# AnyLoc/Revisit-Anything

Measured on AMD Instinct MI355X. Metric: query_images_per_sec, higher is better.
Workload: dtype f32

## Files before the change

revisit-anything_amd/csrc/ctx.h:

```cpp
#pragma once
#include <hip/hip_runtime.h>
#include <math.h>
#include <stdint.h>
#include <stdio.h>
#include <string.h>

#include <map>
#include <string>
#include <vector>

#include "../../include/segvlad.h"

#define SV_HIP(expr)                                                                              \
  do {                                                                                            \
    hipError_t _e = (expr);                                                                       \
    if (_e != hipSuccess) {                                                                       \
      return ctx->fail(SEGVLAD_ERR_HIP, "%s failed: %s (%s:%d)", #expr, hipGetErrorString(_e),    \
                       __FILE__, __LINE__);                                                       \
    }                                                                                             \
  } while (0)

#define SV_TRY(expr)          \
  do {                        \
    int _r = (expr);          \
// ... 277 lines not shown
  if (ctx->desc.open)                                                                                                       \
  return ctx->fail(SEGVLAD_ERR_STATE, what ": a segvlad_describe_begin is open on this context (call segvlad_describe_end first)")

StageTimer* sv_stage_open(segvlad_ctx* ctx, const char* name, int* slot);
struct StageScope {
  segvlad_ctx* ctx;
  StageTimer* t = nullptr;
  int slot = 0;
  StageScope(segvlad_ctx* c, const char* name) : ctx(c) { t = sv_stage_open(c, name, &slot); }
  ~StageScope() { if (t) (void)hipEventRecord(t->ev[2 * slot + 1], ctx->stream); }
  void count(int n = 1) { if (t) t->launches += n; }
};

int sv_launch_vocab_prepare(segvlad_ctx* ctx);
int sv_launch_incidence(segvlad_ctx* ctx, const uint8_t* masks, int S, int Hm, int Wm, int H, int W, int patch,
                        uint64_t* inc_bits, double* centroids );
int sv_launch_centroids(segvlad_ctx* ctx, const uint8_t* masks, int S, int Hm, int Wm, double* out);
bool sv_adjacency_fits(int S_max);
int sv_launch_adjacency(segvlad_ctx* ctx, const double* cent, const int32_t* seg_off_dev, const int64_t* adj_off_dev,
                        int B, int S_max, int order, uint8_t* adj, uint32_t* n_bad, uint8_t* img_flags = nullptr);
int sv_launch_assign(segvlad_ctx* ctx, const float* tokens, int B, int N, float* xt, uint8_t* labels, float* rnorm,
                     float* gap);
int sv_launch_prep(segvlad_ctx* ctx, const uint8_t* labels, const uint64_t* inc_bits, const int32_t* seg_off_dev,
                   const int64_t* adj_off_dev, const uint8_t* adj, int B, int N, int K, int S_max, int SC,
                   uint64_t* colmask, float* gscale, int32_t* phys , int32_t* cov_cnt ,
                   int cover );
int sv_launch_aggregate(segvlad_ctx* ctx, const float* xt, const float* rnorm, const uint8_t* labels,
                        const uint64_t* colmask, const float* centres, int K, int D, const int32_t* seg_off_dev,
                        const float* gscale, int B, int N, int SC, float* out, float* block_norms,
                        const float* mean = nullptr, float xscale = 0.f, uint16_t* h1 = nullptr, uint16_t* h2 = nullptr);

int sv_launch_token_norms(segvlad_ctx* ctx, const float* xt, const uint64_t* colmask, const float* centres, int K, int D,
                          const int32_t* seg_off_dev, int B, int N, int SC, float* block_norms, float xscale, uint16_t* h1,
                          uint16_t* h2, const int32_t* rowbase, int64_t dummy_row ,
                          const int32_t* phys );

int sv_launch_centroid_sums(segvlad_ctx* ctx, const float* xt, const float* rnorm, const uint8_t* labels, int B, int N, int D, int K,
                            double* sums, int64_t* counts);

int sv_launch_row_sumsq(segvlad_ctx* ctx, const float* X, int64_t n, int d, float* out);
int sv_launch_normalize_rows(segvlad_ctx* ctx, const float* X, int64_t n, int d, float* Y);
int sv_launch_gemm_nt(segvlad_ctx* ctx, int mode, const float* A, const float* Bm, float* C, int M, int N, int Kd,
                      int64_t ldc, const float* a_sub, const float* col_scale, const float* row_add,
                      const float* col_add);

int sv_launch_l2_strided(segvlad_ctx* ctx, const float* Q, const float* R, float* dist, int M, int n_sample, int Kd,
                         int64_t ldc, const float* qn, const float* rn, int b_stride, bool split_ok = false);
int sv_launch_l2_strided_parts(segvlad_ctx* ctx, const float* Q, const float* R, float* dist, int M, int n_sample, int Kd,
                               int64_t ldc, const float* qn, const float* rn, int b_stride, const float** parts, int* splits);
int sv_launch_l0_reduce_rank(segvlad_ctx* ctx, const float* parts, int splits, int M, int n_sample, int64_t ldc, const float* qn,
                             const float* rn, int b_stride, int rank, float* thr_out, uint32_t* cand_cnt, const uint32_t* fail_rows);
int sv_launch_l2_filter(segvlad_ctx* ctx, const float* Q, const float* R, int M, int n_sample, int Kd, const float* qn,
                        const float* rn, int b_stride, const float* thr, int64_t thr_ld, uint32_t* cand_cnt,
                        float* cand_d2, uint32_t* cand_id, int cap);

int sv_launch_split_bf16(segvlad_ctx* ctx, const float* X, int64_t n_elems, uint16_t* hi, uint16_t* lo);
int sv_launch_bf16_filter(segvlad_ctx* ctx, const uint16_t* Qh, const uint16_t* Ql, const uint16_t* Rh, const uint16_t* Rl,
                          int M, int n_sample, int d, int b_stride, const float* qn, const float* rn, const float* thr,
                          int64_t thr_ld, float eps_mult, float c_eps, float rn_max, uint32_t* cand_cnt, float* cand_d2,
                          uint32_t* cand_id, int cap);
enum class SvSelect : int { Threshold = 0, Band = 1, Carry = 2 };
struct SvSelectArgs {
  uint32_t* cnt = nullptr;
  float* cd2 = nullptr;
  uint32_t* cid = nullptr;
  int cap = 0;
  int k = 0;
  SvSelect mode = SvSelect::Threshold;
// ... 132 lines not shown
```

revisit-anything_amd/csrc/describe.hip:

```cpp
#include <cmath>
#include "ctx.h"


struct SegWalk { int S_max = 0; bool monotone = true; std::vector<int64_t> adj_off; };
static SegWalk walk_seg_offsets(const int32_t* seg_offsets, int B) {
  SegWalk w;
  w.adj_off.assign((size_t)B + 1, 0);
  for (int b = 0; b < B && w.monotone; ++b) {
    const int s = seg_offsets[b + 1] - seg_offsets[b];
    w.monotone = s >= 0;
    if (s > w.S_max) w.S_max = s;
    w.adj_off[b + 1] = w.adj_off[b] + (int64_t)s * s;
  }
  return w;
}

static int incidence_run(segvlad_ctx* ctx, const uint8_t* masks, int S, int Hm, int Wm, int H, int W, int patch, uint64_t* inc_bits,
                         double* centroids, bool want_centroids) {
  if (S < 0 || Hm <= 0 || Wm <= 0 || H <= 0 || W <= 0 || patch <= 0 || H / patch <= 0 || W / patch <= 0)
    return ctx->fail(SEGVLAD_ERR_ARG, "incidence: bad geometry S=%d masks %dx%d image %dx%d patch %d", S, Hm, Wm, H, W, patch);
  if (S == 0) return SEGVLAD_OK;
  if (!masks || !inc_bits || (want_centroids && !centroids)) return ctx->fail(SEGVLAD_ERR_ARG, "incidence: null pointer");
  const int N = (H / patch) * (W / patch), nw = (N + 63) / 64;
  const void* dm;
// ... 93 lines not shown
  SegWalk w = walk_seg_offsets(io.seg_offsets, B);
  if (!w.monotone) return PLAN_REFUSE(SEGVLAD_ERR_ARG, "images: seg_offsets must be non-decreasing");
  p.S_tot = io.seg_offsets[B], p.S_max = w.S_max, p.SC = w.S_max > 0 ? (w.S_max + 63) / 64 : 1;
  p.adj_off = std::move(w.adj_off);
  const bool plain = pca && !x3;
  const float* y = plain ? nullptr : io.y;
  if (p.S_tot > 0 && (!io.inc_bits || (!io.out && !y && !plain))) return PLAN_REFUSE(SEGVLAD_ERR_ARG, "images: null inc_bits/out");
  p.upload_offsets = passes == Passes::All;
  p.want_desc = p.S_tot > 0 && (io.out || plain), p.want_block_norms = io.block_norms_out && p.S_tot > 0;
  p.want_labels = io.labels_out != nullptr, p.want_gap = io.gap_out != nullptr;
  p.want_y = y != nullptr && p.S_tot > 0;
  if (plain) p.form = DescribeForm::PlainProjection;
  if (!p.want_y) return p;
  const bool project = io.out == nullptr && D % 32 == 0 && ctx->P % 4 == 0 && ctx->opt.pca_path != 1 &&
                       (ctx->opt.pca_path == 2 || ((double)p.S_tot * K >= 1.25 * (double)B * N && (double)B * N >= 128.0 * K));
  p.form = project ? DescribeForm::Project : DescribeForm::Planes;
  p.xscale = sv_fp16_scale(1.f + ctx->pca_mean_maxabs);
  if (!project) return p;
  const float bound = 1.f + ctx->vocab_maxabs;
  if (!std::isfinite(bound)) return PLAN_REFUSE(SEGVLAD_ERR_ARG, "images_pca: the vocabulary holds a non-finite centre");
  p.xscale = sv_fp16_scale(bound);
  p.rows_pad = (((int64_t)B * N + 255) & ~255ll) + 256ll * K;
  if (ctx->pca_w_scale > 0.f) {
    const float zb = std::sqrt((float)D) * (16384.f / ctx->pca_w_scale) * (1.f + ctx->vocab_norm_max);
    if (std::isfinite(zb) && zb > 0.f) p.zscale = sv_fp16_scale(zb);
  }
  return p;
#undef PLAN_REFUSE
}

static int reserve_scratch(segvlad_ctx* ctx, const DescribePlan& p, DescribeIO& io) {
  const size_t B = p.B, N = p.N, D = p.D, K = p.K, P = p.P, S = p.S_tot;
  if (p.form == DescribeForm::Project) {
    SV_HIP(ctx->s_xh1.reserve((size_t)(p.rows_pad + 256) * D * 2));
    SV_HIP(ctx->s_xh2.reserve((size_t)(p.rows_pad + 256) * D * 2));
    SV_HIP(ctx->s_pz.reserve((size_t)p.rows_pad * P * sizeof(float)));
    SV_HIP(ctx->s_rowbase.reserve(B * K * sizeof(int32_t)));
    SV_HIP(ctx->s_tilegrp.reserve((size_t)(p.rows_pad >> 8) * sizeof(int32_t)));
    SV_HIP(ctx->s_phys.reserve(B * N * sizeof(int32_t)));
    SV_HIP(ctx->s_covcnt.reserve(B * K * sizeof(int32_t)));
    SV_HIP(ctx->s_bn.reserve(S * K * sizeof(float)));
  } else if (p.form == DescribeForm::Planes) {
    SV_HIP(ctx->s_xh1.reserve((size_t)sv_x3_rows(p.S_tot) * ctx->KD * 2));
    SV_HIP(ctx->s_xh2.reserve((size_t)sv_x3_rows(p.S_tot) * ctx->KD * 2));
  } else if (p.form == DescribeForm::PlainProjection && !io.out && S > 0) {
    SV_HIP(ctx->s_desc.reserve(S * ctx->KD * sizeof(float)));
    io.out = ctx->s_desc.as<float>();
  }
  SV_HIP(ctx->s_xt.reserve(B * N * D * sizeof(float)));
  SV_HIP(ctx->s_rnorm.reserve(B * N * sizeof(float)));
  if (!p.want_labels) SV_HIP(ctx->s_labels.reserve(B * N));
  if (p.passes == Passes::AssignOnly) return SEGVLAD_OK;
  SV_HIP(ctx->s_colmask.reserve(B * N * p.SC * 8));
  SV_HIP(ctx->s_gscale.reserve((S + 1) * sizeof(float)));
  SV_HIP(ctx->s_segoff.reserve((B + 1) * sizeof(int32_t)));
  SV_HIP(ctx->s_adjoff.reserve((B + 1) * sizeof(int64_t)));
  return SEGVLAD_OK;
}

static int stage_pointers(segvlad_ctx* ctx, const DescribePlan& p, DescribeIO& io) {
  const size_t B = p.B, N = p.N, S = p.S_tot;
  if (p.want_y) SV_TRY(sv_out(ctx, io.y, S * p.P * sizeof(float), &io.d_y));
  SV_TRY(sv_in(ctx, io.tokens, B * p.D * N * sizeof(float), &io.d_tok));
  if (S > 0) SV_TRY(sv_in(ctx, io.inc_bits, S * p.nw * 8, &io.d_inc));
  if (io.adj && S > 0) SV_TRY(sv_in(ctx, io.adj, (size_t)p.adj_off[B], &io.d_adj));
  if (p.want_desc) SV_TRY(sv_out(ctx, io.out, S * p.K * p.D * sizeof(float), &io.d_out));
  if (p.want_labels) SV_TRY(sv_out(ctx, io.labels_out, B * N, &io.d_lab));
  else io.d_lab = ctx->s_labels.p;
// ... 27 lines not shown
  if (!p.l2norm) return SEGVLAD_OK;
  SV_TRY(sv_launch_normalize_rows(ctx, (const float*)io.d_y, p.S_tot, p.P, (float*)io.d_y));
  sc.count();
  return SEGVLAD_OK;
}

static int pass_descriptor(segvlad_ctx* ctx, const DescribePlan& p, const DescribeIO& io) {
  const bool fused = p.form == DescribeForm::Planes;
  uint16_t *h1 = fused ? ctx->s_xh1.as<uint16_t>() : nullptr, *h2 = fused ? ctx->s_xh2.as<uint16_t>() : nullptr;
  {
    StageScope sc(ctx, "aggregate");
    SV_TRY(sv_launch_aggregate(ctx, ctx->s_xt.as<float>(), ctx->s_rnorm.as<float>(), (const uint8_t*)io.d_lab, ctx->s_colmask.as<uint64_t>(),
                               ctx->vocab.as<float>(), p.K, p.D, ctx->s_segoff.as<int32_t>(), ctx->s_gscale.as<float>(), p.B, p.N, p.SC,
                               (float*)io.d_out, (float*)io.d_bn, fused ? ctx->pca_mean.as<float>() : nullptr, p.xscale, h1, h2));
    sc.count();
  }
  if (!fused) return SEGVLAD_OK;
  StageScope sc(ctx, "pca");
  SV_TRY(sv_launch_gemm_f16x3(ctx, h1, h2, ctx->pca_w1.as<uint16_t>(), ctx->pca_w2.as<uint16_t>(), p.S_tot, p.P, ctx->KD,
                              1.f / (p.xscale * ctx->pca_w_scale), ctx->pca_scale.as<float>(), (float*)io.d_y));
  sc.count(2);
  return pass_normalize(ctx, p, io, sc);
}

static int pass_project(segvlad_ctx* ctx, const DescribePlan& p, const DescribeIO& io) {
  float* bn = io.d_bn ? (float*)io.d_bn : ctx->s_bn.as<float>();
  uint16_t *h1 = ctx->s_xh1.as<uint16_t>(), *h2 = ctx->s_xh2.as<uint16_t>();
  {
    StageScope sc(ctx, "aggregate");
    SV_TRY(sv_launch_group_plan(ctx, ctx->s_covcnt.as<int32_t>(), p.B, p.K, ctx->s_rowbase.as<int32_t>(), ctx->s_tilegrp.as<int32_t>(),
                                (int)(p.rows_pad >> 8)));
    SV_TRY(sv_launch_token_norms(ctx, ctx->s_xt.as<float>(), ctx->s_colmask.as<uint64_t>(), ctx->vocab.as<float>(), p.K, p.D,
                                 ctx->s_segoff.as<int32_t>(), p.B, p.N, p.SC, bn, p.xscale, h1, h2, ctx->s_rowbase.as<int32_t>(),
                                 ctx->opt.debug_search == 7 ? -p.rows_pad : p.rows_pad, ctx->s_phys.as<int32_t>()));
    sc.count(2);
  }
  StageScope sc(ctx, "pca");
  SV_TRY(sv_launch_gemm_f16x3_grouped(ctx, h1, h2, ctx->pca_w1.as<uint16_t>(), ctx->pca_w2.as<uint16_t>(), (int)p.rows_pad, p.P, p.D, p.K,
                                      ctx->s_tilegrp.as<int32_t>(), 1.f / (p.xscale * ctx->pca_w_scale), ctx->s_pz.as<float>()));
  SV_TRY(sv_launch_project_aggregate(ctx, ctx->s_pz.as<float>(), ctx->pca_cproj.as<float>(), bn, ctx->s_gscale.as<float>(),
                                     ctx->s_colmask.as<uint64_t>(), ctx->s_laboff.as<int32_t>(), ctx->s_rowbase.as<int32_t>(),
                                     ctx->s_phys.as<int32_t>(), ctx->s_segoff.as<int32_t>(), p.B, p.N, p.K, p.P, p.SC, p.S_max,
                                     ctx->pca_scale.as<float>(), (float*)io.d_y, p.zscale));
  sc.count(2);
  return pass_normalize(ctx, p, io, sc);
}

static int join_mask_branch(segvlad_ctx* ctx) {
  if (!ctx->desc.side_pending) return SEGVLAD_OK;
  ctx->desc.side_pending = false;
  return sv_join_side(ctx);
}
static int run_describe(segvlad_ctx* ctx, const DescribePlan& p, DescribeIO& io) {
  SV_TRY(reserve_scratch(ctx, p, io));
  if (p.form == DescribeForm::Project && !ctx->pca_cproj_valid) {
    SV_HIP(ctx->pca_cproj.reserve((size_t)ctx->P * sizeof(float)));
    SV_TRY(sv_launch_project_consts(ctx, ctx->pca_comps.as<float>(), ctx->pca_mean.as<float>(), ctx->P, ctx->KD, ctx->pca_cproj.as<float>()));
    ctx->pca_cproj_valid = true;
  }
  SV_TRY(stage_pointers(ctx, p, io));
  if (p.passes != Passes::FromPrep) SV_TRY(pass_assign(ctx, p, io));
  if (p.passes == Passes::AssignOnly) return SEGVLAD_OK;
  SV_TRY(join_mask_branch(ctx));
  if (p.S_tot == 0) return SEGVLAD_OK;
  SV_TRY(pass_prep(ctx, p, io));
  return p.form == DescribeForm::Project ? pass_project(ctx, p, io) : pass_descriptor(ctx, p, io);
}
// ... 271 lines not shown
```

revisit-anything_amd/csrc/vlad_kernels.hip:

```cpp
#include <stdio.h>
#include <stdlib.h>

#include "ctx.h"
#include "incidence_dev.h"

typedef float f32x16 __attribute__((ext_vector_type(16)));

#define MFMA32(a, b, c) __builtin_amdgcn_mfma_f32_32x32x2f32((a), (b), (c), 0, 0, 0)

template <int CTRL>
__device__ __forceinline__ float dpp_f32(float x) {
  return __int_as_float(__builtin_amdgcn_update_dpp(0, __float_as_int(x), CTRL, 0xf, 0xf, true));
}

__device__ __forceinline__ int frag_row(int r, int kk) { return (r & 3) + 8 * (r >> 2) + 4 * kk; }

__global__ void vocab_norm_kernel(const float* __restrict__ C, int K, int D, float* __restrict__ inv) {
  const int k = blockIdx.x;
  float s = 0.f;
  for (int d = threadIdx.x; d < D; d += blockDim.x) {
    float v = C[(size_t)k * D + d];
    s = fmaf(v, v, s);
  }
  __shared__ float red[256];
// ... 991 lines not shown
            const size_t o = (size_t)(s0 + 64 * sc + row) * KD + (size_t)k * D + dcol;
            if ((!PLANES || out != nullptr) && ABL != 2) *reinterpret_cast<float4*>(out + o) = v;
            if (PLANES && ABL != 2) {
              typedef _Float16 h4 __attribute__((ext_vector_type(4)));
              const float f[4] = {(v.x - mu4.x) * xscale, (v.y - mu4.y) * xscale, (v.z - mu4.z) * xscale, (v.w - mu4.w) * xscale};
              h4 p1, p2;
#pragma unroll
              for (int e = 0; e < 4; ++e) {
                p1[e] = (_Float16)f[e];
                p2[e] = (_Float16)(f[e] - (float)p1[e]);
              }
              const size_t ob = sv_x3_off(s0 + 64 * sc + row, (int64_t)k * D + dcol, KD);
              *reinterpret_cast<h4*>(h1 + ob) = p1;
              *reinterpret_cast<h4*>(h2 + ob) = p2;
            }
          }
        }
      }
    }
    SV_APHASE(3)
    __syncthreads();
    SV_APHASE(4)
  }
  }
}

constexpr int TNK_QD = 8, TNK_LCAP = 256, TNK_WAVES = 4;

__device__ __forceinline__ void tnk_wait_vm(int n) {
#define TNK_W(v) case v: asm volatile("s_waitcnt vmcnt(" #v ")" ::: "memory"); break;
  switch (n) {
    TNK_W(0) TNK_W(1) TNK_W(2) TNK_W(3) TNK_W(4) TNK_W(5) TNK_W(6) TNK_W(7) TNK_W(8) TNK_W(9) TNK_W(10) TNK_W(11)
    TNK_W(12) TNK_W(13) TNK_W(14) TNK_W(15) TNK_W(16) TNK_W(17) TNK_W(18) TNK_W(19) TNK_W(20) TNK_W(21) TNK_W(22)
    default: asm volatile("s_waitcnt vmcnt(23)" ::: "memory"); break;
  }
#undef TNK_W
}

template <bool BIG>
__global__ __launch_bounds__(64 * TNK_WAVES, 2) void token_norms_kernel(const float* __restrict__ Xt, const float* __restrict__ rnorm,
                                                                    const int32_t* __restrict__ tok_order,
                                                                    const int32_t* __restrict__ lab_off,
                                                                    const uint64_t* __restrict__ colmask,
                                                                    const float* __restrict__ C,
                                                                    const int32_t* __restrict__ seg_off, int N, int D, int K, int SC,
                                                                    int Dpad, float* __restrict__ block_norms, float xscale,
                                                                    _Float16* __restrict__ h1, _Float16* __restrict__ h2,
                                                                    const int32_t* __restrict__ rowbase, int64_t dummy_row,
                                                                    int skip_le, const uint8_t* __restrict__ redo_task,
                                                                    const int32_t* __restrict__ phys) {
  extern __shared__ __attribute__((aligned(16))) unsigned char smem[];
  const int b = blockIdx.y;
  const int tid = threadIdx.x, l = tid & 63, i = l & 31, kk = l >> 5;
  const int w = __builtin_amdgcn_readfirstlane(tid >> 6);
  const int k = (int)blockIdx.x * TNK_WAVES + w;
  if (k >= K) return;
  const size_t wsz = (size_t)TNK_QD * 1024 + (size_t)TNK_LCAP * 20 + (size_t)Dpad * 4;
  unsigned char* qbase = smem + (size_t)w * wsz;
  uint64_t* mskl = reinterpret_cast<uint64_t*>(qbase + TNK_QD * 1024);
  int* tokl = reinterpret_cast<int*>(mskl + TNK_LCAP);
  float* rnl = reinterpret_cast<float*>(tokl + TNK_LCAP);
  int* rowl = reinterpret_cast<int*>(rnl + TNK_LCAP);
  float* cl = reinterpret_cast<float*>(rowl + TNK_LCAP);
  const int o0 = lab_off[(size_t)b * (K + 1) + k];
  const int n = lab_off[(size_t)b * (K + 1) + k + 1] - o0;
  const int s0 = seg_off[b], S = seg_off[b + 1] - s0;
  const int SCb = (S + 63) >> 6;
  const int npairs = (n + 1) >> 1;
  const int nd = Dpad >> 7, total = nd * npairs;
  const size_t tb = (size_t)b * N + o0;
  if ((n >= TNK_LCAP) != BIG) return;
  if (n <= skip_le && !(redo_task && n > 0 && redo_task[(size_t)b * K + k])) return;
  if (n == 0) {
    for (int s = l; s < S; s += 64) block_norms[(size_t)(s0 + s) * K + k] = 0.f;
    return;
  }
  for (int d = 4 * l; d < Dpad; d += 256)
    *reinterpret_cast<float4*>(cl + d) = d < D ? *reinterpret_cast<const float4*>(C + (size_t)k * D + d) : make_float4(0.f, 0.f, 0.f, 0.f);
  constexpr bool single = !BIG;
  const int grow0 = rowbase[(size_t)b * K + k];
  if (single) {
    for (int j = l; j < n; j += 64) {
      tokl[j] = tok_order[tb + j];
      rnl[j] = rnorm[tb + j];
      const int ph = phys[tb + j];
      rowl[j] = ph >= 0 ? grow0 + ph : -1;
    }
    if (l == 0 && (n & 1)) {
      tokl[n] = 0;
      rnl[n] = 0.f;
      rowl[n] = -1;
    }
  }
  const size_t nkb_d = (size_t)(D >> 5);
  const size_t ob_dummy = sv_x3_off((dummy_row < 0 ? -dummy_row : dummy_row) + ((64 * k + l) & 255), (4 * i) % D, D);
  const float* Xb = Xt + (size_t)b * N * D;

  for (int sc = 0; sc < SCb; ++sc) {
    if (single) {
      for (int j = l; j < n; j += 64) mskl[j] = colmask[(tb + j) * SC + sc];
      if (l == 0 && (n & 1)) mskl[n] = 0;
    }
    const int Sc = min(64, S - 64 * sc);
    const bool two = Sc > 32;
    f32x16 acc[2][4];
    float nsq[2][16];
#pragma unroll
    for (int a = 0; a < 2; ++a)
#pragma unroll
      for (int r = 0; r < 16; ++r) {
        nsq[a][r] = 0.f;
#pragma unroll
        for (int q = 0; q < 4; ++q) acc[a][q][r] = 0.f;
      }
    int idc = 0, ip = 0, fi = 0;
    auto issue = [&]() {
      const int j = 2 * ip + kk;
      const int t = single ? lds_read_i32(lds_addr(tokl + j)) : (j < n ? tok_order[tb + j] : 0);
      const int dcol = idc * 128 + 4 * i;
      const float* src = dcol < D ? Xb + (size_t)t * D + dcol : Xt;
      __builtin_amdgcn_global_load_lds((agg_gptr_t)src, (agg_lptr_t)(qbase + (fi % TNK_QD) * 1024), 16, 0, 0);
      ++fi;
      if (++ip == npairs) {
        ip = 0;
        ++idc;
      }
    };
    for (int q = 0; q < TNK_QD && q < total; ++q) issue();
    int f = 0;
    for (int dc = 0; dc < nd; ++dc) {
      const int dcol = dc * 128 + 4 * i;
      const bool dvalid = dcol < D;
      const f32x4 c4 = lds_read_f32x4(lds_addr(cl + dcol));
      const size_t kb_dc = (size_t)(dcol >> 5);
      const unsigned lane_c = (unsigned)((dcol & 31) >> 3), lane_o = (unsigned)(dcol & 7);
      for (int p = 0; p < npairs; ++p, ++f) {
        const int j = 2 * p + kk;
        float rn = 0.f;
        uint64_t m = 0ull;
        f32x4 x;
        int prw = -1;
        if (!single) {
          rn = j < n ? rnorm[tb + j] : 0.f;
          m = j < n ? colmask[(tb + j) * SC + sc] : 0ull;
          const int ph = (sc == 0 && j < n) ? phys[tb + j] : -1;
          prw = ph >= 0 ? grow0 + ph : -1;
        }
        const int rem = total - 1 - f;
        if (single && dummy_row >= 0) {
          if (f >= TNK_QD && rem >= TNK_QD - 1) {
            if (sc == 0) asm volatile("s_waitcnt vmcnt(23)" ::: "memory");
            else asm volatile("s_waitcnt vmcnt(7)" ::: "memory");
          } else {
            tnk_wait_vm((rem < TNK_QD - 1 ? rem : TNK_QD - 1) + (sc == 0 ? 2 * (f < TNK_QD ? f : TNK_QD) : 0));
          }
        } else {
          asm volatile("s_waitcnt vmcnt(0)" ::: "memory");
        }
        if (single)
          lds_step_read(lds_addr(qbase + (f % TNK_QD) * 1024 + l * 16), lds_addr(rnl + j), lds_addr(mskl + j), x, rn, m);
        else
          x = lds_read_f32x4(lds_addr(qbase + (f % TNK_QD) * 1024 + l * 16));
        if (fi < total) issue();
        if (!dvalid) x = f32x4{0.f, 0.f, 0.f, 0.f};
        const float b0 = fmaf(x.x, rn, -c4.x), b1 = fmaf(x.y, rn, -c4.y);
        const float b2 = fmaf(x.z, rn, -c4.z), b3 = fmaf(x.w, rn, -c4.w);
        if (sc == 0) {
          typedef _Float16 h4 __attribute__((ext_vector_type(4)));
          const float fv[4] = {b0 * xscale, b1 * xscale, b2 * xscale, b3 * xscale};
          h4 p1, p2;
#pragma unroll
          for (int e = 0; e < 4; ++e) {
            p1[e] = (_Float16)fv[e];
            p2[e] = (_Float16)(fv[e] - (float)p1[e]);
          }
          if (single) prw = lds_read_i32(lds_addr(rowl + j));
          const bool real = dvalid && prw >= 0;
          const unsigned rr = (unsigned)prw;
          const size_t ob = real ? ((size_t)(rr >> 7) * nkb_d + kb_dc) * 4096 + (size_t)(((rr & 127u) << 5) + (((lane_c ^ (unsigned)sv_x3_swz(rr)) << 3) | lane_o))
                                 : ob_dummy;
          *reinterpret_cast<h4*>(h1 + ob) = p1;
          *reinterpret_cast<h4*>(h2 + ob) = p2;
        }
        const float a0 = ((m >> i) & 1ull) ? 1.f : 0.f;
        acc[0][0] = MFMA32(a0, b0, acc[0][0]);
        acc[0][1] = MFMA32(a0, b1, acc[0][1]);
        acc[0][2] = MFMA32(a0, b2, acc[0][2]);
        acc[0][3] = MFMA32(a0, b3, acc[0][3]);
        if (two) {
          const float a1 = ((m >> (32 + i)) & 1ull) ? 1.f : 0.f;
          acc[1][0] = MFMA32(a1, b0, acc[1][0]);
          acc[1][1] = MFMA32(a1, b1, acc[1][1]);
          acc[1][2] = MFMA32(a1, b2, acc[1][2]);
          acc[1][3] = MFMA32(a1, b3, acc[1][3]);
        }
      }
#pragma unroll
      for (int mt = 0; mt < 2; ++mt) {
        if (mt == 1 && !two) break;
#pragma unroll
        for (int r = 0; r < 16; ++r) {
          float q2 = nsq[mt][r];
#pragma unroll
          for (int q = 0; q < 4; ++q) {
            q2 = fmaf(acc[mt][q][r], acc[mt][q][r], q2);
            acc[mt][q][r] = 0.f;
          }
          nsq[mt][r] = q2;
        }
      }
    }
#pragma unroll
    for (int mt = 0; mt < 2; ++mt) {
      if (mt == 1 && !two) break;
#pragma unroll
      for (int r = 0; r < 16; ++r) {
        float p = nsq[mt][r];
        p += dpp_f32<0xB1>(p);
        p += dpp_f32<0x4E>(p);
        p += dpp_f32<0x141>(p);
        p += dpp_f32<0x140>(p);
        p += __shfl_xor(p, 16);
        const int row = 32 * mt + frag_row(r, kk);
        if (i == 0 && row < Sc) block_norms[(size_t)(s0 + 64 * sc + row) * K + k] = sqrtf(p);
      }
    }
  }
}

constexpr int GNK_SLOT = 4096;

template <int T, int QS>
__global__ __launch_bounds__(T == 1 ? 256 : 128, 2) void gram_norms_kernel(const float* __restrict__ Xt, const float* __restrict__ rnorm,
                                                                         const int32_t* __restrict__ tok_order,
                                                                         const int32_t* __restrict__ lab_off,
                                                                         const uint64_t* __restrict__ colmask,
                                                                         const float* __restrict__ C,
                                                                         const int32_t* __restrict__ seg_off, int N, int D, int K, int SC,
                                                                         float* __restrict__ block_norms, float xscale,
                                                                         _Float16* __restrict__ h1, _Float16* __restrict__ h2,
                                                                         const int32_t* __restrict__ rowbase, int safe_waits,
                                                                         uint8_t* __restrict__ redo_task,
                                                                         const int32_t* __restrict__ phys, int64_t dummy_row) {
  extern __shared__ __attribute__((aligned(16))) unsigned char smem[];
  typedef _Float16 f16x8 __attribute__((ext_vector_type(8)));
  constexpr int WAVES = T == 1 ? 4 : 2;
  constexpr int NG = T * (T + 1) / 2;
  const int b = blockIdx.y;
  const int tid = threadIdx.x, l = tid & 63, i = l & 31, kk = l >> 5;
  const int w = __builtin_amdgcn_readfirstlane(tid >> 6);
  const int k = (int)blockIdx.x * WAVES + w;
  if (k >= K) return;
  const size_t wsz = (size_t)QS * T * GNK_SLOT + (size_t)D * 4;
  unsigned char* qbase = smem + (size_t)w * wsz;
  float* cl = reinterpret_cast<float*>(qbase + QS * T * GNK_SLOT);
  const int o0 = lab_off[(size_t)b * (K + 1) + k];
  const int n = lab_off[(size_t)b * (K + 1) + k + 1] - o0;
  if (n > 32 * T || (T == 2 && n <= 32)) return;
  const int s0 = seg_off[b], S = seg_off[b + 1] - s0;
  if (n == 0) {
    for (int s = l; s < S; s += 64) block_norms[(size_t)(s0 + s) * K + k] = 0.f;
    return;
  }
  const size_t tb = (size_t)b * N + o0;
  for (int d = 4 * l; d < D; d += 256) *reinterpret_cast<float4*>(cl + d) = *reinterpret_cast<const float4*>(C + (size_t)k * D + d);
  bool real[T];
  float rn[T];
#pragma unroll
  for (int tt = 0; tt < T; ++tt) {
    real[tt] = 32 * tt + i < n;
    rn[tt] = real[tt] ? rnorm[tb + 32 * tt + i] : 0.f;
  }
  const float* Xb = Xt + (size_t)b * N * D;
  const float* src[4 * T];
#pragma unroll
  for (int pz = 0; pz < 4 * T; ++pz) {
    const int jj = 8 * pz + (l >> 3);
    const int t = jj < n ? tok_order[tb + jj] : tok_order[tb];
    src[pz] = Xb + (size_t)t * D + 4 * ((l & 7) ^ ((jj >> 1) & 7));
  }
  const int steps = D >> 5;
  const int NP = (n + 7) >> 3;
  auto issue = [&](int f) {
#pragma unroll
    for (int pz = 0; pz < 4 * T; ++pz)
      if (pz < NP) {
        if (8 * pz + (l >> 3) < n)
          __builtin_amdgcn_global_load_lds((agg_gptr_t)(src[pz] + 32 * f), (agg_lptr_t)(qbase + (f % QS) * (T * GNK_SLOT) + pz * 1024), 16, 0, 0);
      }
  };
#pragma unroll
  for (int q = 0; q < QS; ++q)
    if (q < steps) issue(q);
  f32x16 acc[NG];
#pragma unroll
  for (int g = 0; g < NG; ++g)
#pragma unroll
    for (int r = 0; r < 16; ++r) acc[g][r] = 0.f;
  size_t prow[T];
  unsigned pswz[T];
#pragma unroll
  for (int tt = 0; tt < T; ++tt) {
    const int ph = real[tt] ? phys[tb + 32 * tt + i] : 0;
    const int64_t rr = ph >= 0 ? (int64_t)rowbase[(size_t)b * K + k] + ph : dummy_row + ((32 * (k + tt) + i) & 255);
    prow[tt] = (size_t)(rr >> 7) * (size_t)(D >> 5) * 4096 + (size_t)(rr & 127) * 32;
    pswz[tt] = (unsigned)sv_x3_swz(rr);
  }
  const unsigned fsw = (unsigned)((i >> 1) & 7);
  const unsigned a_tok = lds_addr(qbase) + (unsigned)i * 128u;
  for (int f = 0; f < steps; ++f) {
    if (f >= QS && f + QS - 1 < steps && !safe_waits) tnk_wait_vm(QS * 4 * T + (QS - 1) * NP);
    else asm volatile("s_waitcnt vmcnt(0)" ::: "memory");
    f32x4 x[T][4], c[4];
    {
      const unsigned ac = lds_addr(cl) + (unsigned)(32 * f + 8 * kk) * 4u;
      const unsigned p0 = ((unsigned)(2 * kk) ^ fsw) << 4, p1 = ((unsigned)(2 * kk + 1) ^ fsw) << 4;
      const unsigned p2 = ((unsigned)(4 + 2 * kk) ^ fsw) << 4, p3 = ((unsigned)(5 + 2 * kk) ^ fsw) << 4;
#pragma unroll
      for (int tt = 0; tt < T; ++tt) {
        const unsigned a0 = a_tok + (unsigned)(f % QS) * (T * GNK_SLOT) + (unsigned)tt * GNK_SLOT;
        asm volatile("ds_read_b128 %0, %4\n\tds_read_b128 %1, %5\n\tds_read_b128 %2, %6\n\tds_read_b128 %3, %7"
                     : "=&v"(x[tt][0]), "=&v"(x[tt][1]), "=&v"(x[tt][2]), "=&v"(x[tt][3])
                     : "v"(a0 + p0), "v"(a0 + p1), "v"(a0 + p2), "v"(a0 + p3)
                     : "memory");
      }
      asm volatile("ds_read_b128 %0, %4\n\tds_read_b128 %1, %4 offset:16\n\tds_read_b128 %2, %4 offset:64\n\tds_read_b128 %3, %4 offset:80\n\t"
                   "s_waitcnt lgkmcnt(0)"
                   : "=&v"(c[0]), "=&v"(c[1]), "=&v"(c[2]), "=&v"(c[3])
                   : "v"(ac)
                   : "memory");
#pragma unroll
      for (int tt = 0; tt < T; ++tt) asm volatile("" : "+v"(x[tt][0]), "+v"(x[tt][1]), "+v"(x[tt][2]), "+v"(x[tt][3]));
    }
    if (f + QS < steps) issue(f + QS);
    asm volatile("" ::: "memory");
#pragma unroll
    for (int ks = 0; ks < 2; ++ks) {
      f16x8 hh[T], ll[T];
#pragma unroll
      for (int tt = 0; tt < T; ++tt) {
#pragma unroll
        for (int e = 0; e < 8; ++e) {
          const float xv = x[tt][2 * ks + (e >> 2)][e & 3], cv = c[2 * ks + (e >> 2)][e & 3];
          const float fv = real[tt] ? fmaf(xv, rn[tt], -cv) * xscale : 0.f;
          hh[tt][e] = (_Float16)fv;
          ll[tt][e] = (_Float16)(fv - (float)hh[tt][e]);
        }
        const size_t ob = prow[tt] + (size_t)f * 4096 + (size_t)((((unsigned)(2 * ks + kk)) ^ pswz[tt]) << 3);
        if (real[tt]) {
          *reinterpret_cast<f16x8*>(h1 + ob) = hh[tt];
          *reinterpret_cast<f16x8*>(h2 + ob) = ll[tt];
        }
      }
#pragma unroll
      for (int ta = 0, g = 0; ta < T; ++ta)
#pragma unroll
        for (int tb2 = ta; tb2 < T; ++tb2, ++g) {
          acc[g] = __builtin_amdgcn_mfma_f32_32x32x16_f16(ll[ta], hh[tb2], acc[g], 0, 0, 0);
          acc[g] = __builtin_amdgcn_mfma_f32_32x32x16_f16(hh[ta], ll[tb2], acc[g], 0, 0, 0);
          acc[g] = __builtin_amdgcn_mfma_f32_32x32x16_f16(hh[ta], hh[tb2], acc[g], 0, 0, 0);
        }
    }
  }
  float dgl[T];
#pragma unroll
  for (int tt = 0; tt < T; ++tt) {
    dgl[tt] = 0.f;
    const int gd = tt == 0 ? 0 : NG - 1;
#pragma unroll
    for (int r = 0; r < 16; ++r)
      if (frag_row(r, kk) == i) dgl[tt] = acc[gd][r];
  }
  bool cancels = false;
  const float inv_x2 = 1.f / (xscale * xscale);
  const int SCb = (S + 63) >> 6;
  for (int sc = 0; sc < SCb; ++sc) {
    const int Sc = min(64, S - 64 * sc);
    uint64_t mt[T];
#pragma unroll
    for (int tt = 0; tt < T; ++tt) mt[tt] = real[tt] ? colmask[(tb + 32 * tt + i) * SC + sc] : 0ull;
    for (int s = 0; s < Sc; ++s) {
      uint32_t W[T];
      bool any = false;
#pragma unroll
      for (int tt = 0; tt < T; ++tt) {
        W[tt] = (uint32_t)__builtin_amdgcn_ballot_w64(((mt[tt] >> s) & 1ull) != 0ull);
        any |= W[tt] != 0u;
      }
      float p = 0.f;
      if (any) {
#pragma unroll
        for (int ta = 0, g = 0; ta < T; ++ta)
#pragma unroll
          for (int tb2 = ta; tb2 < T; ++tb2, ++g) {
            float q = 0.f;
#pragma unroll
            for (int r = 0; r < 16; ++r) q += ((W[ta] >> frag_row(r, kk)) & 1u) ? acc[g][r] : 0.f;
            q = ((W[tb2] >> i) & 1u) ? q : 0.f;
            p += (ta == tb2) ? q : 2.f * q;
          }
        p += dpp_f32<0xB1>(p);
        p += dpp_f32<0x4E>(p);
        p += dpp_f32<0x141>(p);
        p += dpp_f32<0x140>(p);
        p += __shfl_xor(p, 16);
        p += __shfl_xor(p, 32);
        float dg = 0.f;
#pragma unroll
        for (int tt = 0; tt < T; ++tt) dg += ((W[tt] >> i) & 1u) ? dgl[tt] : 0.f;
        dg += dpp_f32<0xB1>(dg);
        dg += dpp_f32<0x4E>(dg);
        dg += dpp_f32<0x141>(dg);
        dg += dpp_f32<0x140>(dg);
        dg += __shfl_xor(dg, 16);
        dg += __shfl_xor(dg, 32);
        cancels = cancels || (p < 0.0625f * dg);
      }
      if (l == 0) block_norms[(size_t)(s0 + 64 * sc + s) * K + k] = sqrtf(fmaxf(p, 0.f) * inv_x2);
    }
  }
  if (cancels && l == 0 && redo_task) redo_task[(size_t)b * K + k] = 1;
}

int sv_launch_token_norms(segvlad_ctx* ctx, const float* xt, const uint64_t* colmask, const float* centres, int K, int D,
                          const int32_t* seg_off_dev, int B, int N, int SC, float* block_norms, float xscale, uint16_t* h1,
                          uint16_t* h2, const int32_t* rowbase, int64_t dummy_row, const int32_t* phys) {
  if (D % 4) return ctx->fail(SEGVLAD_ERR_ARG, "token_norms: D=%d must be a multiple of 4", D);
  const int Dpad = (D + 127) & ~127;
  const size_t lds = (size_t)TNK_WAVES * ((size_t)TNK_QD * 1024 + (size_t)TNK_LCAP * 20 + (size_t)Dpad * 4);
  if (lds > 160 * 1024) return ctx->fail(SEGVLAD_ERR_LIMIT, "token_norms: D=%d needs %zu B of LDS", D, lds);
  const bool gram = ctx->opt.tnk_gram != 0 && (D % 32) == 0;
  const int skip_le = gram ? 64 : -1;
  uint8_t* redo_task = nullptr;
  if (gram) {
    SV_HIP(ctx->s_tnk_redo.reserve((size_t)B * K));
    redo_task = ctx->s_tnk_redo.as<uint8_t>();
    SV_HIP(hipMemsetAsync(redo_task, 0, (size_t)B * K, ctx->stream));
    const bool fork = N > 32 && ctx->opt.tnk_fork != 0;
    if (fork) SV_TRY(sv_fork_side(ctx));
    for (int T = 2; T >= 1; --T) {
      if (T == 2 && N <= 32) continue;
      const int waves = T == 1 ? 4 : 2;
      const int qs = T == 1 ? 3 : 2;
      const size_t glds = (size_t)waves * ((size_t)qs * T * GNK_SLOT + (size_t)D * 4);
      auto gk = T == 1 ? gram_norms_kernel<1, 3> : gram_norms_kernel<2, 2>;
      if (glds > 64 * 1024) SV_HIP(sv_max_dyn_lds(reinterpret_cast<const void*>(gk), glds));
      hipLaunchKernelGGL(gk, dim3((K + waves - 1) / waves, B), dim3(64 * waves), glds, (T == 2 && fork) ? ctx->side : ctx->stream, xt,
                         ctx->s_rnsorted.as<float>(), ctx->s_tokorder.as<int32_t>(), ctx->s_laboff.as<int32_t>(), colmask, centres,
                         seg_off_dev, N, D, K, SC, block_norms, xscale, reinterpret_cast<_Float16*>(h1),
                         reinterpret_cast<_Float16*>(h2), rowbase, dummy_row < 0 ? 1 : 0, redo_task, phys,
                         dummy_row < 0 ? -dummy_row : dummy_row);
      SV_HIP(hipGetLastError());
    }
    if (fork) SV_TRY(sv_join_side(ctx));
  }
  for (int big = 0; big < 2; ++big) {
    if (big && N < TNK_LCAP) break;
    auto kern = big ? token_norms_kernel<true> : token_norms_kernel<false>;
    if (lds > 64 * 1024)
      SV_HIP(sv_max_dyn_lds(reinterpret_cast<const void*>(kern), (size_t)lds));
    hipLaunchKernelGGL(kern, dim3((K + TNK_WAVES - 1) / TNK_WAVES, B), dim3(64 * TNK_WAVES), lds, ctx->stream, xt,
                       ctx->s_rnsorted.as<float>(), ctx->s_tokorder.as<int32_t>(), ctx->s_laboff.as<int32_t>(), colmask, centres,
                       seg_off_dev, N, D, K, SC, Dpad, block_norms, xscale, reinterpret_cast<_Float16*>(h1),
                       reinterpret_cast<_Float16*>(h2), rowbase, dummy_row, skip_le, redo_task, phys);
    SV_HIP(hipGetLastError());
  }
  return SEGVLAD_OK;
}

int sv_launch_aggregate(segvlad_ctx* ctx, const float* xt, const float* ,
                        const uint8_t* ,
                        const uint64_t* colmask, const float* centres, int K, int D, const int32_t* seg_off_dev,
                        const float* gscale, int B, int N, int SC, float* out, float* block_norms, const float* mean,
                        float xscale, uint16_t* h1, uint16_t* h2) {
  const int nwaves = (D + 127) / 128;
  if (nwaves > 12)
    return ctx->fail(SEGVLAD_ERR_LIMIT, "aggregate: D=%d exceeds the 1536-wide workgroup of this build", D);
  const int Ncap = (N + 2) & ~1;
  const int PW = nwaves * 2 + 1;
  size_t lds = (size_t)Ncap * 16 + (size_t)(64 * PW + 64) * sizeof(float) + 16 * sizeof(int);
  lds = (lds + 15) & ~(size_t)15;
  lds += (size_t)nwaves * 6 * 1024;
  if (lds > 160 * 1024) return ctx->fail(SEGVLAD_ERR_LIMIT, "aggregate: N=%d tokens need %zu B of LDS (limit 160 KiB)", N, lds);
  auto kern = (h1 != nullptr) ? aggregate_kernel<true> : aggregate_kernel<false>;
  bool phases = false;
#ifdef SEGVLAD_ABLATIONS
  if (const char* ab = getenv("SEGVLAD_AGG_ABL")) {
    if (atoi(ab) == 1) kern = aggregate_kernel<false, 1>;
    if (atoi(ab) == 2) kern = aggregate_kernel<false, 2>;
    if (atoi(ab) == 9) {
      kern = aggregate_kernel<false, 9>;
      phases = true;
      unsigned long long z[8] = {0, 0, 0, 0, 0, 0, 0, 0};
      SV_HIP(hipMemcpyToSymbol(HIP_SYMBOL(sv_agg_phase_cycles), z, sizeof(z)));
    }
  }
#endif
// ... 26 lines not shown
```

Baseline: 8884.

## Drop dummy-row fp16 plane stores and share centre tile across batch waves

Token-norm and gram-norm kernels no longer write placeholder rows for uncovered tokens. Stores and loads are issued only when some lane in the wave has a real row, and the vmcnt wait counts are computed from how many stores and loads were actually issued. The gram kernel's grid is transposed so each workgroup handles one centre across several images, which lets the centre vector be loaded into LDS once per block instead of once per wave. The scratch padding that existed for dummy rows is removed, in exchange for more complex wait-count bookkeeping and a ballot on every store.

```diff
diff --git a/revisit-anything_amd/csrc/ctx.h b/revisit-anything_amd/csrc/ctx.h
--- a/revisit-anything_amd/csrc/ctx.h
+++ b/revisit-anything_amd/csrc/ctx.h
@@ -333,8 +333,7 @@
 
 int sv_launch_token_norms(segvlad_ctx* ctx, const float* xt, const uint64_t* colmask, const float* centres, int K, int D,
                           const int32_t* seg_off_dev, int B, int N, int SC, float* block_norms, float xscale, uint16_t* h1,
-                          uint16_t* h2, const int32_t* rowbase, int64_t dummy_row ,
-                          const int32_t* phys );
+                          uint16_t* h2, const int32_t* rowbase, const int32_t* phys );
 
 int sv_launch_centroid_sums(segvlad_ctx* ctx, const float* xt, const float* rnorm, const uint8_t* labels, int B, int N, int D, int K,
                             double* sums, int64_t* counts);
diff --git a/revisit-anything_amd/csrc/describe.hip b/revisit-anything_amd/csrc/describe.hip
--- a/revisit-anything_amd/csrc/describe.hip
+++ b/revisit-anything_amd/csrc/describe.hip
@@ -149,8 +149,8 @@
 static int reserve_scratch(segvlad_ctx* ctx, const DescribePlan& p, DescribeIO& io) {
   const size_t B = p.B, N = p.N, D = p.D, K = p.K, P = p.P, S = p.S_tot;
   if (p.form == DescribeForm::Project) {
-    SV_HIP(ctx->s_xh1.reserve((size_t)(p.rows_pad + 256) * D * 2));
-    SV_HIP(ctx->s_xh2.reserve((size_t)(p.rows_pad + 256) * D * 2));
+    SV_HIP(ctx->s_xh1.reserve((size_t)p.rows_pad * D * 2));
+    SV_HIP(ctx->s_xh2.reserve((size_t)p.rows_pad * D * 2));
     SV_HIP(ctx->s_pz.reserve((size_t)p.rows_pad * P * sizeof(float)));
     SV_HIP(ctx->s_rowbase.reserve(B * K * sizeof(int32_t)));
     SV_HIP(ctx->s_tilegrp.reserve((size_t)(p.rows_pad >> 8) * sizeof(int32_t)));
@@ -244,7 +244,7 @@
                                 (int)(p.rows_pad >> 8)));
     SV_TRY(sv_launch_token_norms(ctx, ctx->s_xt.as<float>(), ctx->s_colmask.as<uint64_t>(), ctx->vocab.as<float>(), p.K, p.D,
                                  ctx->s_segoff.as<int32_t>(), p.B, p.N, p.SC, bn, p.xscale, h1, h2, ctx->s_rowbase.as<int32_t>(),
-                                 ctx->opt.debug_search == 7 ? -p.rows_pad : p.rows_pad, ctx->s_phys.as<int32_t>()));
+                                 ctx->s_phys.as<int32_t>()));
     sc.count(2);
   }
   StageScope sc(ctx, "pca");
diff --git a/revisit-anything_amd/csrc/vlad_kernels.hip b/revisit-anything_amd/csrc/vlad_kernels.hip
--- a/revisit-anything_amd/csrc/vlad_kernels.hip
+++ b/revisit-anything_amd/csrc/vlad_kernels.hip
@@ -1047,7 +1047,8 @@
   switch (n) {
     TNK_W(0) TNK_W(1) TNK_W(2) TNK_W(3) TNK_W(4) TNK_W(5) TNK_W(6) TNK_W(7) TNK_W(8) TNK_W(9) TNK_W(10) TNK_W(11)
     TNK_W(12) TNK_W(13) TNK_W(14) TNK_W(15) TNK_W(16) TNK_W(17) TNK_W(18) TNK_W(19) TNK_W(20) TNK_W(21) TNK_W(22)
-    default: asm volatile("s_waitcnt vmcnt(23)" ::: "memory"); break;
+    TNK_W(23) TNK_W(24) TNK_W(25) TNK_W(26) TNK_W(27) TNK_W(28) TNK_W(29) TNK_W(30)
+    default: asm volatile("s_waitcnt vmcnt(31)" ::: "memory"); break;
   }
 #undef TNK_W
 }
@@ -1061,7 +1062,7 @@
                                                                     const int32_t* __restrict__ seg_off, int N, int D, int K, int SC,
                                                                     int Dpad, float* __restrict__ block_norms, float xscale,
                                                                     _Float16* __restrict__ h1, _Float16* __restrict__ h2,
-                                                                    const int32_t* __restrict__ rowbase, int64_t dummy_row,
+                                                                    const int32_t* __restrict__ rowbase, int safe_waits,
                                                                     int skip_le, const uint8_t* __restrict__ redo_task,
                                                                     const int32_t* __restrict__ phys) {
   extern __shared__ __attribute__((aligned(16))) unsigned char smem[];
@@ -1108,7 +1109,6 @@
     }
   }
   const size_t nkb_d = (size_t)(D >> 5);
-  const size_t ob_dummy = sv_x3_off((dummy_row < 0 ? -dummy_row : dummy_row) + ((64 * k + l) & 255), (4 * i) % D, D);
   const float* Xb = Xt + (size_t)b * N * D;
 
   for (int sc = 0; sc < SCb; ++sc) {
@@ -1129,6 +1129,7 @@
         for (int q = 0; q < 4; ++q) acc[a][q][r] = 0.f;
       }
     int idc = 0, ip = 0, fi = 0;
+    uint32_t stored = 0u;
     auto issue = [&]() {
       const int j = 2 * ip + kk;
       const int t = single ? lds_read_i32(lds_addr(tokl + j)) : (j < n ? tok_order[tb + j] : 0);
@@ -1162,12 +1163,12 @@
           prw = ph >= 0 ? grow0 + ph : -1;
         }
         const int rem = total - 1 - f;
-        if (single && dummy_row >= 0) {
-          if (f >= TNK_QD && rem >= TNK_QD - 1) {
+        if (single && !safe_waits) {
+          if (f >= TNK_QD && rem >= TNK_QD - 1 && (sc != 0 || stored == (1u << TNK_QD) - 1u)) {
             if (sc == 0) asm volatile("s_waitcnt vmcnt(23)" ::: "memory");
             else asm volatile("s_waitcnt vmcnt(7)" ::: "memory");
           } else {
-            tnk_wait_vm((rem < TNK_QD - 1 ? rem : TNK_QD - 1) + (sc == 0 ? 2 * (f < TNK_QD ? f : TNK_QD) : 0));
+            tnk_wait_vm((rem < TNK_QD - 1 ? rem : TNK_QD - 1) + (sc == 0 ? 2 * __builtin_popcount(stored) : 0));
           }
         } else {
           asm volatile("s_waitcnt vmcnt(0)" ::: "memory");
@@ -1191,11 +1192,17 @@
           }
           if (single) prw = lds_read_i32(lds_addr(rowl + j));
           const bool real = dvalid && prw >= 0;
-          const unsigned rr = (unsigned)prw;
-          const size_t ob = real ? ((size_t)(rr >> 7) * nkb_d + kb_dc) * 4096 + (size_t)(((rr & 127u) << 5) + (((lane_c ^ (unsigned)sv_x3_swz(rr)) << 3) | lane_o))
-                                 : ob_dummy;
-          *reinterpret_cast<h4*>(h1 + ob) = p1;
-          *reinterpret_cast<h4*>(h2 + ob) = p2;
+          const bool some = __builtin_amdgcn_ballot_w64(real) != 0ull;
+          if (some) {
+            asm volatile("" ::: "memory");
+            if (real) {
+              const unsigned rr = (unsigned)prw;
+              const size_t ob = ((size_t)(rr >> 7) * nkb_d + kb_dc) * 4096 + (size_t)(((rr & 127u) << 5) + (((lane_c ^ (unsigned)sv_x3_swz(rr)) << 3) | lane_o));
+              *reinterpret_cast<h4*>(h1 + ob) = p1;
+              *reinterpret_cast<h4*>(h2 + ob) = p2;
+            }
+          }
+          stored = ((stored << 1) | (some ? 1u : 0u)) & ((1u << TNK_QD) - 1u);
         }
         const float a0 = ((m >> i) & 1ull) ? 1.f : 0.f;
         acc[0][0] = MFMA32(a0, b0, acc[0][0]);
@@ -1251,56 +1258,70 @@
                                                                          const int32_t* __restrict__ lab_off,
                                                                          const uint64_t* __restrict__ colmask,
                                                                          const float* __restrict__ C,
-                                                                         const int32_t* __restrict__ seg_off, int N, int D, int K, int SC,
-                                                                         float* __restrict__ block_norms, float xscale,
+                                                                         const int32_t* __restrict__ seg_off, int B, int N, int D, int K,
+                                                                         int SC, float* __restrict__ block_norms, float xscale,
                                                                          _Float16* __restrict__ h1, _Float16* __restrict__ h2,
                                                                          const int32_t* __restrict__ rowbase, int safe_waits,
                                                                          uint8_t* __restrict__ redo_task,
-                                                                         const int32_t* __restrict__ phys, int64_t dummy_row) {
+                                                                         const int32_t* __restrict__ phys) {
   extern __shared__ __attribute__((aligned(16))) unsigned char smem[];
   typedef _Float16 f16x8 __attribute__((ext_vector_type(8)));
   constexpr int WAVES = T == 1 ? 4 : 2;
   constexpr int NG = T * (T + 1) / 2;
-  const int b = blockIdx.y;
+  const int k = blockIdx.x;
   const int tid = threadIdx.x, l = tid & 63, i = l & 31, kk = l >> 5;
   const int w = __builtin_amdgcn_readfirstlane(tid >> 6);
-  const int k = (int)blockIdx.x * WAVES + w;
-  if (k >= K) return;
-  const size_t wsz = (size_t)QS * T * GNK_SLOT + (size_t)D * 4;
-  unsigned char* qbase = smem + (size_t)w * wsz;
-  float* cl = reinterpret_cast<float*>(qbase + QS * T * GNK_SLOT);
+  const int b = (int)blockIdx.y * WAVES + w;
+  unsigned char* qbase = smem + (size_t)w * (QS * T * GNK_SLOT);
+  float* cl = reinterpret_cast<float*>(smem + (size_t)WAVES * QS * T * GNK_SLOT);
+  for (int d = 4 * tid; d < D; d += 256 * WAVES) *reinterpret_cast<float4*>(cl + d) = *reinterpret_cast<const float4*>(C + (size_t)k * D + d);
+  __syncthreads();
+  if (b >= B) return;
   const int o0 = lab_off[(size_t)b * (K + 1) + k];
   const int n = lab_off[(size_t)b * (K + 1) + k + 1] - o0;
   if (n > 32 * T || (T == 2 && n <= 32)) return;
   const int s0 = seg_off[b], S = seg_off[b + 1] - s0;
-  if (n == 0) {
+  const size_t tb = (size_t)b * N + o0;
+  bool cov[T];
+  int ph[T];
+  float rn[T];
+  uint32_t tmask = 0u, pmask = 0u, lpen = 0u;
+#pragma unroll
+  for (int tt = 0; tt < T; ++tt) {
+    ph[tt] = 32 * tt + i < n ? phys[tb + 32 * tt + i] : -1;
+    cov[tt] = ph[tt] >= 0;
+    rn[tt] = cov[tt] ? rnorm[tb + 32 * tt + i] : 0.f;
+    if (__builtin_amdgcn_ballot_w64(cov[tt]) != 0ull) tmask |= 1u << tt;
+  }
+#pragma unroll
+  for (int pz = 0; pz < 4 * T; ++pz) {
+    const int jj = 8 * pz + (l >> 3);
+    const bool pc = jj < n && phys[tb + jj] >= 0;
+    if (pc) lpen |= 1u << pz;
+    if (__builtin_amdgcn_ballot_w64(pc) != 0ull) pmask |= 1u << pz;
+  }
+  tmask = (uint32_t)__builtin_amdgcn_readfirstlane((int)tmask);
+  pmask = (uint32_t)__builtin_amdgcn_readfirstlane((int)pmask);
+  if (tmask == 0u) {
     for (int s = l; s < S; s += 64) block_norms[(size_t)(s0 + s) * K + k] = 0.f;
     return;
   }
-  const size_t tb = (size_t)b * N + o0;
-  for (int d = 4 * l; d < D; d += 256) *reinterpret_cast<float4*>(cl + d) = *reinterpret_cast<const float4*>(C + (size_t)k * D + d);
-  bool real[T];
-  float rn[T];
-#pragma unroll
-  for (int tt = 0; tt < T; ++tt) {
-    real[tt] = 32 * tt + i < n;
-    rn[tt] = real[tt] ? rnorm[tb + 32 * tt + i] : 0.f;
-  }
   const float* Xb = Xt + (size_t)b * N * D;
   const float* src[4 * T];
 #pragma unroll
   for (int pz = 0; pz < 4 * T; ++pz) {
     const int jj = 8 * pz + (l >> 3);
-    const int t = jj < n ? tok_order[tb + jj] : tok_order[tb];
+    const int t = ((lpen >> pz) & 1u) ? tok_order[tb + jj] : 0;
     src[pz] = Xb + (size_t)t * D + 4 * ((l & 7) ^ ((jj >> 1) & 7));
   }
   const int steps = D >> 5;
-  const int NP = (n + 7) >> 3;
+  const int NPI = __builtin_popcount(pmask), NST = 4 * __builtin_popcount(tmask);
   auto issue = [&](int f) {
 #pragma unroll
     for (int pz = 0; pz < 4 * T; ++pz)
-      if (pz < NP) {
-        if (8 * pz + (l >> 3) < n)
+      if ((pmask >> pz) & 1u) {
+        asm volatile("" ::: "memory");
+        if ((lpen >> pz) & 1u)
           __builtin_amdgcn_global_load_lds((agg_gptr_t)(src[pz] + 32 * f), (agg_lptr_t)(qbase + (f % QS) * (T * GNK_SLOT) + pz * 1024), 16, 0, 0);
       }
   };
@@ -1316,15 +1337,14 @@
   unsigned pswz[T];
 #pragma unroll
   for (int tt = 0; tt < T; ++tt) {
-    const int ph = real[tt] ? phys[tb + 32 * tt + i] : 0;
-    const int64_t rr = ph >= 0 ? (int64_t)rowbase[(size_t)b * K + k] + ph : dummy_row + ((32 * (k + tt) + i) & 255);
+    const int64_t rr = cov[tt] ? (int64_t)rowbase[(size_t)b * K + k] + ph[tt] : 0;
     prow[tt] = (size_t)(rr >> 7) * (size_t)(D >> 5) * 4096 + (size_t)(rr & 127) * 32;
     pswz[tt] = (unsigned)sv_x3_swz(rr);
   }
   const unsigned fsw = (unsigned)((i >> 1) & 7);
   const unsigned a_tok = lds_addr(qbase) + (unsigned)i * 128u;
   for (int f = 0; f < steps; ++f) {
-    if (f >= QS && f + QS - 1 < steps && !safe_waits) tnk_wait_vm(QS * 4 * T + (QS - 1) * NP);
+    if (f >= QS && f + QS - 1 < steps && !safe_waits) tnk_wait_vm(QS * NST + (QS - 1) * NPI);
     else asm volatile("s_waitcnt vmcnt(0)" ::: "memory");
     f32x4 x[T][4], c[4];
     {
@@ -1357,14 +1377,17 @@
 #pragma unroll
         for (int e = 0; e < 8; ++e) {
           const float xv = x[tt][2 * ks + (e >> 2)][e & 3], cv = c[2 * ks + (e >> 2)][e & 3];
-          const float fv = real[tt] ? fmaf(xv, rn[tt], -cv) * xscale : 0.f;
+          const float fv = cov[tt] ? fmaf(xv, rn[tt], -cv) * xscale : 0.f;
           hh[tt][e] = (_Float16)fv;
           ll[tt][e] = (_Float16)(fv - (float)hh[tt][e]);
         }
-        const size_t ob = prow[tt] + (size_t)f * 4096 + (size_t)((((unsigned)(2 * ks + kk)) ^ pswz[tt]) << 3);
-        if (real[tt]) {
-          *reinterpret_cast<f16x8*>(h1 + ob) = hh[tt];
-          *reinterpret_cast<f16x8*>(h2 + ob) = ll[tt];
+        if ((tmask >> tt) & 1u) {
+          asm volatile("" ::: "memory");
+          if (cov[tt]) {
+            const size_t ob = prow[tt] + (size_t)f * 4096 + (size_t)((((unsigned)(2 * ks + kk)) ^ pswz[tt]) << 3);
+            *reinterpret_cast<f16x8*>(h1 + ob) = hh[tt];
+            *reinterpret_cast<f16x8*>(h2 + ob) = ll[tt];
+          }
         }
       }
 #pragma unroll
@@ -1393,7 +1416,7 @@
     const int Sc = min(64, S - 64 * sc);
     uint64_t mt[T];
 #pragma unroll
-    for (int tt = 0; tt < T; ++tt) mt[tt] = real[tt] ? colmask[(tb + 32 * tt + i) * SC + sc] : 0ull;
+    for (int tt = 0; tt < T; ++tt) mt[tt] = cov[tt] ? colmask[(tb + 32 * tt + i) * SC + sc] : 0ull;
     for (int s = 0; s < Sc; ++s) {
       uint32_t W[T];
       bool any = false;
@@ -1439,13 +1462,14 @@
 
 int sv_launch_token_norms(segvlad_ctx* ctx, const float* xt, const uint64_t* colmask, const float* centres, int K, int D,
                           const int32_t* seg_off_dev, int B, int N, int SC, float* block_norms, float xscale, uint16_t* h1,
-                          uint16_t* h2, const int32_t* rowbase, int64_t dummy_row, const int32_t* phys) {
+                          uint16_t* h2, const int32_t* rowbase, const int32_t* phys) {
   if (D % 4) return ctx->fail(SEGVLAD_ERR_ARG, "token_norms: D=%d must be a multiple of 4", D);
   const int Dpad = (D + 127) & ~127;
   const size_t lds = (size_t)TNK_WAVES * ((size_t)TNK_QD * 1024 + (size_t)TNK_LCAP * 20 + (size_t)Dpad * 4);
   if (lds > 160 * 1024) return ctx->fail(SEGVLAD_ERR_LIMIT, "token_norms: D=%d needs %zu B of LDS", D, lds);
   const bool gram = ctx->opt.tnk_gram != 0 && (D % 32) == 0;
   const int skip_le = gram ? 64 : -1;
+  const int safe_waits = ctx->opt.debug_search == 7 ? 1 : 0;
   uint8_t* redo_task = nullptr;
   if (gram) {
     SV_HIP(ctx->s_tnk_redo.reserve((size_t)B * K));
@@ -1457,14 +1481,14 @@
       if (T == 2 && N <= 32) continue;
       const int waves = T == 1 ? 4 : 2;
       const int qs = T == 1 ? 3 : 2;
-      const size_t glds = (size_t)waves * ((size_t)qs * T * GNK_SLOT + (size_t)D * 4);
+      const size_t glds = (size_t)waves * qs * T * GNK_SLOT + (size_t)D * 4;
+      if (glds > 160 * 1024) return ctx->fail(SEGVLAD_ERR_LIMIT, "token_norms: D=%d needs %zu B of LDS", D, glds);
       auto gk = T == 1 ? gram_norms_kernel<1, 3> : gram_norms_kernel<2, 2>;
       if (glds > 64 * 1024) SV_HIP(sv_max_dyn_lds(reinterpret_cast<const void*>(gk), glds));
-      hipLaunchKernelGGL(gk, dim3((K + waves - 1) / waves, B), dim3(64 * waves), glds, (T == 2 && fork) ? ctx->side : ctx->stream, xt,
+      hipLaunchKernelGGL(gk, dim3(K, (B + waves - 1) / waves), dim3(64 * waves), glds, (T == 2 && fork) ? ctx->side : ctx->stream, xt,
                          ctx->s_rnsorted.as<float>(), ctx->s_tokorder.as<int32_t>(), ctx->s_laboff.as<int32_t>(), colmask, centres,
-                         seg_off_dev, N, D, K, SC, block_norms, xscale, reinterpret_cast<_Float16*>(h1),
-                         reinterpret_cast<_Float16*>(h2), rowbase, dummy_row < 0 ? 1 : 0, redo_task, phys,
-                         dummy_row < 0 ? -dummy_row : dummy_row);
+                         seg_off_dev, B, N, D, K, SC, block_norms, xscale, reinterpret_cast<_Float16*>(h1),
+                         reinterpret_cast<_Float16*>(h2), rowbase, safe_waits, redo_task, phys);
       SV_HIP(hipGetLastError());
     }
     if (fork) SV_TRY(sv_join_side(ctx));
@@ -1477,7 +1501,7 @@
     hipLaunchKernelGGL(kern, dim3((K + TNK_WAVES - 1) / TNK_WAVES, B), dim3(64 * TNK_WAVES), lds, ctx->stream, xt,
                        ctx->s_rnsorted.as<float>(), ctx->s_tokorder.as<int32_t>(), ctx->s_laboff.as<int32_t>(), colmask, centres,
                        seg_off_dev, N, D, K, SC, Dpad, block_norms, xscale, reinterpret_cast<_Float16*>(h1),
-                       reinterpret_cast<_Float16*>(h2), rowbase, dummy_row, skip_le, redo_task, phys);
+                       reinterpret_cast<_Float16*>(h2), rowbase, safe_waits, skip_le, redo_task, phys);
     SV_HIP(hipGetLastError());
   }
   return SEGVLAD_OK;
```

Result: no change. 8926, median of 6 (+0.5%).
